# yang-0201/MAF-YOLO

Measured on AMD Instinct MI355X. Metric: images/sec MAF-YOLO-n 640x640 bs=32 infer (Model.forward + non_max_suppression), higher is better.
Workload: dtype f16

## Files before the change

### maf-yolo_amd/csrc/bottleneck.hip

```cpp
#include "maf_common.h"
#include "lds_pipe.h"

namespace {

struct BnArgs {
    const half_t* x; half_t* out;
    const unsigned char* par;
    const float* b2;
    int B, H, W, Cin, Cout, nMB, x_stride, x_coff, out_stride, out_coff;
    int tilesX, tilesY, nwg;
    int ko;
    const half_t* xs[3];
    int xs_stride[3], xs_coff[3];
    const unsigned char* w3;
    int C3, nx;
    unsigned* ctr;
    int ntiles;
    unsigned long long* prof;
};

#ifdef MAF_BN_PROFILE
#define BN_KO(bit) ((a.ko >> (bit)) & 1)
#else
#define BN_KO(bit) 0
#endif
#ifdef MAF_BN_STAMPS
#define BN_STAMP(i) do { uint64_t now_; asm volatile("s_memtime %0\n\ts_waitcnt lgkmcnt(0)" : "=s"(now_) :: "memory"); prof_acc[i] += (uint32_t)(now_ - prof_t); prof_t = now_; } while (0)
#else
#define BN_STAMP(i) do { } while (0)
#endif

typedef half_t half4v_t __attribute__((ext_vector_type(4)));


__device__ __forceinline__ float bn_silu2(float v) { return v * __builtin_amdgcn_rcpf(1.f + __builtin_amdgcn_exp2f(-v)); }
__device__ __forceinline__ void bn_silu2_pk4(float v0, float v1, float v2, float v3, half2_t& o01, half2_t& o23) {
    const half2_t xa = {(half_t)v0, (half_t)v1}, xb = {(half_t)v2, (half_t)v3};
    const uint32_t ua = __builtin_bit_cast(uint32_t, xa), ub = __builtin_bit_cast(uint32_t, xb);
    uint32_t ea, eb, ra, rb;
    asm("v_exp_f16_sdwa %0, -%1 dst_sel:WORD_0 dst_unused:UNUSED_PAD src0_sel:WORD_0" : "=v"(ea) : "v"(ua));
    asm("v_exp_f16_sdwa %0, -%1 dst_sel:WORD_0 dst_unused:UNUSED_PAD src0_sel:WORD_0" : "=v"(eb) : "v"(ub));
    asm("v_exp_f16_sdwa %0, -%1 dst_sel:WORD_1 dst_unused:UNUSED_PRESERVE src0_sel:WORD_1" : "+v"(ea) : "v"(ua));
    asm("v_exp_f16_sdwa %0, -%1 dst_sel:WORD_1 dst_unused:UNUSED_PRESERVE src0_sel:WORD_1" : "+v"(eb) : "v"(ub));
    const half2_t one = {(half_t)1.f, (half_t)1.f};
    const uint32_t da = __builtin_bit_cast(uint32_t, __builtin_bit_cast(half2_t, ea) + one), db = __builtin_bit_cast(uint32_t, __builtin_bit_cast(half2_t, eb) + one);
    asm("v_rcp_f16_sdwa %0, %1 dst_sel:WORD_0 dst_unused:UNUSED_PAD src0_sel:WORD_0" : "=v"(ra) : "v"(da));
    asm("v_rcp_f16_sdwa %0, %1 dst_sel:WORD_0 dst_unused:UNUSED_PAD src0_sel:WORD_0" : "=v"(rb) : "v"(db));
    asm("v_rcp_f16_sdwa %0, %1 dst_sel:WORD_1 dst_unused:UNUSED_PRESERVE src0_sel:WORD_1" : "+v"(ra) : "v"(da));
    asm("v_rcp_f16_sdwa %0, %1 dst_sel:WORD_1 dst_unused:UNUSED_PRESERVE src0_sel:WORD_1" : "+v"(rb) : "v"(db));
    o01 = xa * __builtin_bit_cast(half2_t, ra);
    o23 = xb * __builtin_bit_cast(half2_t, rb);
}
#ifdef MAF_BN_PERSIST
constexpr bool BN_PERSIST = true;
#else
constexpr bool BN_PERSIST = false;
#endif
#ifdef MAF_BN_PKSILU
constexpr bool BN_PK = true;
#else
constexpr bool BN_PK = false;
#endif

template <int K, int S1, int CT2>
struct BnCfg {
    static constexpr int P = K / 2, PARTS = K > 5 ? 2 : 1;
    static constexpr int RH = 16 + K - 1;
    static constexpr int RWC = (16 + K - 1 + 3) & ~3;
    static constexpr int NHP = RH * RWC, NPT = (NHP + 15) / 16;
    static constexpr int MT = (NPT + 3) / 4;
    static constexpr int RWP = 24;
    static constexpr int PSB = ((RH * RWP * 2 - 8 + 255) / 256) * 256 + 8;
    static constexpr int PS = PSB / 2;
    static constexpr int NTOE = 8 * K * PARTS * 16;
    static constexpr int OFF_W1 = 0, OFF_B1 = 2 * S1 * 1024, REC_A = OFF_B1 + 128;
    static constexpr int OFF_TOE = REC_A, OFF_W2 = OFF_TOE + NTOE * 16, OFF_BD = OFF_W2 + CT2 * 1024;
    static constexpr int REC = OFF_BD + 128;
    static constexpr int REC_B = REC - REC_A;
#ifdef MAF_BN_OCC3
    static constexpr bool OCC3 = true;
#else
    static constexpr bool OCC3 = false;
#endif
    static constexpr bool ZT = CT2 == 4 && K <= 5 && !OCC3;
    static constexpr bool DB = !OCC3;
    static constexpr size_t LDS = (size_t)32 * PSB + (size_t)REC + (DB ? (size_t)REC_B : 0) + (ZT ? (size_t)NTOE * 16 : 0);
    static constexpr int ZOFF = REC + (DB ? REC_B : 0);
};

template <int K, int S1, int CT2, int C3T = 0, int NX = 0>
__global__ __launch_bounds__(256, ((CT2 == 2 && K <= 5) || (BnCfg<K, S1, CT2>::OCC3 && K <= 5)) ? 3 : 2) void bottleneck_kernel(const BnArgs a) {
    typedef BnCfg<K, S1, CT2> Cf;
    constexpr int P = Cf::P, PARTS = Cf::PARTS, RWC = Cf::RWC, NHP = Cf::NHP, NPT = Cf::NPT, MT = Cf::MT, RWP = Cf::RWP, PS = Cf::PS;
    extern __shared__ __attribute__((aligned(16))) unsigned char smem_raw[];
    half_t* T1 = reinterpret_cast<half_t*>(smem_raw);
    unsigned char* rec = smem_raw + 32 * Cf::PSB;

    const int tid = threadIdx.x, wave = tid >> 6, lane = tid & 63, g = lane >> 4, p = lane & 15;
    int lid;
    __shared__ int s_next;
    const int my_xcd = blockIdx.x & 7;
    const int seg_q = a.ntiles >> 3, seg_r = a.ntiles & 7;
    auto seg_start = [&](int x) { return x < seg_r ? x * (seg_q + 1) : seg_r * (seg_q + 1) + (x - seg_r) * seg_q; };
    auto seg_stat = [&](int x) { return ((int)gridDim.x >> 3) + (x < ((int)gridDim.x & 7) ? 1 : 0); };
    auto fetch_tile = [&]() -> int {
        const int j = seg_stat(my_xcd) + (int)atomicAdd(a.ctr + my_xcd, 1u);
        return j < seg_q + (my_xcd < seg_r ? 1 : 0) ? seg_start(my_xcd) + j : -1;
    };
    {
        const int bid = blockIdx.x, xcd = bid & 7, j = bid >> 3;
        const int q = a.ntiles >> 3, r = a.ntiles & 7;
        lid = (xcd < r ? xcd * (q + 1) : r * (q + 1) + (xcd - r) * q) + j;
    }
    bool first_tile = true;
    for (;;) {
    int tid_l = threadIdx.x;
    if constexpr (BN_PERSIST) asm volatile("" : "+v"(tid_l));
    const int tid = tid_l, wave = tid >> 6, lane = tid & 63, g = lane >> 4, p = lane & 15;
    int next_tile = -1;
    if (BN_PERSIST && tid == 0) next_tile = fetch_tile();
    const int tx = lid % a.tilesX;
    const int tt = lid / a.tilesX;
    const int ty = tt % a.tilesY;
    const int b = tt / a.tilesY;
    const int y0 = ty * 16, x0 = tx * 16;
    const half_t* xin = a.x + (size_t)b * a.H * a.W * a.x_stride + a.x_coff;

    const int cg0 = g * 8 < a.Cin ? g * 8 : 0;
    const int cg1 = 32 + g * 8 < a.Cin ? 32 + g * 8 : 0;
    uint32_t xoff[MT];
#pragma unroll
    for (int i = 0; i < MT; ++i) {
        const int m = (wave + 4 * i) * 16 + p;
        const int hr = m / RWC, hc = m - hr * RWC;
        const int iy = min(max(y0 - P + hr, 0), a.H - 1), ix = min(max(x0 - P + hc, 0), a.W - 1);
        xoff[i] = (uint32_t)(iy * a.W + ix) * a.x_stride;
    }
    int ko_block = 0;
#ifndef MAF_BN_XD
#define MAF_BN_XD 3
#endif
    constexpr int XD = Cf::OCC3 ? 1 : (MAF_BN_XD < MT ? MAF_BN_XD : MT - 1);
    half8_t af[XD + 1][S1];
    auto load_x = [&](auto idx) {
        constexpr int i = decltype(idx)::value;
        if constexpr (i < MT) {
            if (BN_KO(0) && ko_block > 0) return;
            af[i % (XD + 1)][0] = *reinterpret_cast<const half8_t*>(xin + xoff[i] + cg0);
            if constexpr (S1 > 1) af[i % (XD + 1)][1] = *reinterpret_cast<const half8_t*>(xin + xoff[i] + cg1);
        }
    };
    auto load_x_head = [&]() {
        maf_static_for<XD>([&](auto idx) { load_x(idx); });
    };
    const bool interior = y0 - P >= 0 && x0 - P >= 0 && y0 - P + Cf::RH <= a.H && x0 - P + RWC <= a.W;
    constexpr int MTH = Cf::OCC3 ? 1 : MT;
    uint32_t tmlo[MTH], tmhi[MTH];
    int tdst[MTH];
#pragma unroll
    for (int i = 0; i < (Cf::OCC3 ? 0 : MT); ++i) {
        const int m0 = (wave + 4 * i) * 16 + g * 4;
        const int hr = m0 / RWC, hc0 = m0 - hr * RWC;
        tmlo[i] = tmhi[i] = 0xffffffffu;
        if (!interior) {
            const int iy = y0 - P + hr, ixb = x0 - P + hc0;
            const bool rowok = (unsigned)iy < (unsigned)a.H;
            const uint32_t k0 = (rowok && (unsigned)(ixb + 0) < (unsigned)a.W) ? 0x0000ffffu : 0u, k1 = (rowok && (unsigned)(ixb + 1) < (unsigned)a.W) ? 0xffff0000u : 0u;
            const uint32_t k2 = (rowok && (unsigned)(ixb + 2) < (unsigned)a.W) ? 0x0000ffffu : 0u, k3 = (rowok && (unsigned)(ixb + 3) < (unsigned)a.W) ? 0xffff0000u : 0u;
            tmlo[i] = k0 | k1; tmhi[i] = k2 | k3;
        }
        tdst[i] = m0 < NHP ? p * PS + hr * RWP + hc0 : -1;
    }
    auto dma_part = [&](int mb, int off, int bytes, int dst) {
        const unsigned char* src = a.par + (size_t)mb * Cf::REC + off;
        const int nvec = bytes >> 4;
        for (int v0 = wave * 64; v0 < nvec; v0 += 256) {
            if (v0 + lane < nvec)
                __builtin_amdgcn_global_load_lds((const void __attribute__((address_space(1)))*)(src + (size_t)(v0 + lane) * 16),
                                                 (void __attribute__((address_space(3)))*)(rec + dst + v0 * 16), 16, 0, 0);
        }
    };

    f32x4_t acc2[4][CT2];
#pragma unroll
    for (int i = 0; i < 4; ++i)
#pragma unroll
        for (int ct = 0; ct < CT2; ++ct) acc2[i][ct] = (f32x4_t)0.f;

    const uint32_t toe_mask = (p >> 2) == g ? 0xffffffffu : 0u;
    const int q4 = wave * 4;
    int hi_off = 4;
    asm volatile("" : "+v"(hi_off));

#ifdef MAF_BN_STAMPS
    uint32_t prof_acc[8] = {0, 0, 0, 0, 0, 0, 0, 0};
    uint64_t prof_t;
    asm volatile("s_memtime %0\n\ts_waitcnt lgkmcnt(0)" : "=s"(prof_t) :: "memory");
#endif
    dma_part(0, 0, Cf::REC, 0);
    load_x_head();
    if constexpr (Cf::ZT) {
        if (first_tile) {
            u32x4_t* z = reinterpret_cast<u32x4_t*>(rec + Cf::ZOFF);
            for (int i = tid; i < Cf::NTOE; i += 256) z[i] = (u32x4_t){0u, 0u, 0u, 0u};
        }
    }
    __syncthreads();
    BN_STAMP(0);

    for (int mb = 0; mb < a.nMB; ++mb) {
        ko_block = mb;
        if (!Cf::DB && mb > 0) dma_part(mb, Cf::REC_A, Cf::REC_B, Cf::REC_A);
        const unsigned char* recB = rec + (Cf::DB ? (mb & 1) * Cf::REC_B : 0);
        if (!BN_KO(8)) {
            half8_t w1f[2][S1];
#pragma unroll
            for (int ct = 0; ct < 2; ++ct)
#pragma unroll
                for (int ks = 0; ks < S1; ++ks) w1f[ct][ks] = reinterpret_cast<const half8_t*>(rec + Cf::OFF_W1)[(ct * S1 + ks) * 64 + lane];
            const float b1v0 = reinterpret_cast<const float*>(rec + Cf::OFF_B1)[p], b1v1 = reinterpret_cast<const float*>(rec + Cf::OFF_B1)[16 + p];
            f32x4_t accn[2];
            auto mma_tile = [&](auto idx) {
                constexpr int i = decltype(idx)::value;
                if constexpr (i < MT) {
                    accn[0] = (f32x4_t)b1v0; accn[1] = (f32x4_t)b1v1;
#pragma unroll
                    for (int ks = 0; ks < S1; ++ks)
#pragma unroll
                        for (int ct = 0; ct < 2; ++ct) {
                            const half8_t wv = Cf::OCC3 ? reinterpret_cast<const half8_t*>(rec + Cf::OFF_W1)[(ct * S1 + ks) * 64 + lane] : w1f[ct][ks];
                            accn[ct] = __builtin_amdgcn_mfma_f32_16x16x32_f16(af[i % (XD + 1)][ks], wv, accn[ct], 0, 0, 0);
                        }
                }
            };
            if constexpr (!Cf::OCC3) mma_tile(std::integral_constant<int, 0>{});
            maf_static_for<MT>([&](auto idx) {
                constexpr int i = decltype(idx)::value;
                const int t = wave + 4 * i;
                load_x(std::integral_constant<int, i + XD>{});
                if constexpr (Cf::OCC3) mma_tile(idx);
                f32x4_t acc1[2] = {accn[0], accn[1]};
                if constexpr (!Cf::OCC3) mma_tile(std::integral_constant<int, i + 1>{});
                __builtin_amdgcn_sched_barrier(0);
                uint32_t mlo, mhi;
                int doff;
                if constexpr (!Cf::OCC3) {
                    mlo = tmlo[i]; mhi = tmhi[i]; doff = tdst[i];
                } else {
                    const int m0 = t * 16 + g * 4;
                    const int hr = m0 / RWC, hc0 = m0 - hr * RWC;
                    mlo = mhi = 0xffffffffu;
                    if (!interior) {
                        const int iy = y0 - P + hr, ixb = x0 - P + hc0;
                        const bool rowok = (unsigned)iy < (unsigned)a.H;
                        mlo = ((rowok && (unsigned)(ixb + 0) < (unsigned)a.W) ? 0x0000ffffu : 0u) | ((rowok && (unsigned)(ixb + 1) < (unsigned)a.W) ? 0xffff0000u : 0u);
                        mhi = ((rowok && (unsigned)(ixb + 2) < (unsigned)a.W) ? 0x0000ffffu : 0u) | ((rowok && (unsigned)(ixb + 3) < (unsigned)a.W) ? 0xffff0000u : 0u);
                    }
                    doff = m0 < NHP ? p * PS + hr * RWP + hc0 : -1;
                }
                half_t* dst = T1 + doff;
#pragma unroll
                for (int ct = 0; ct < 2; ++ct) {
                    half2_t h01, h23;
                    if (BN_KO(1)) {
                        h01 = half2_t{(half_t)acc1[ct][0], (half_t)acc1[ct][1]}; h23 = half2_t{(half_t)acc1[ct][2], (half_t)acc1[ct][3]};
                    } else if constexpr (BN_PK) {
                        bn_silu2_pk4(acc1[ct][0], acc1[ct][1], acc1[ct][2], acc1[ct][3], h01, h23);
                    } else {
                        h01 = half2_t{(half_t)bn_silu2(acc1[ct][0]), (half_t)bn_silu2(acc1[ct][1])};
                        h23 = half2_t{(half_t)bn_silu2(acc1[ct][2]), (half_t)bn_silu2(acc1[ct][3])};
                    }
                    const u32x2_t w = {__builtin_bit_cast(uint32_t, h01) & mlo, __builtin_bit_cast(uint32_t, h23) & mhi};
                    if (doff >= 0 && !BN_KO(4)) *reinterpret_cast<u32x2_t*>(dst + (size_t)(16 * ct) * PS) = w;
                }
            });
        }
        BN_STAMP(1);
        if (!BN_KO(7)) __syncthreads();
        BN_STAMP(2);
        if (mb + 1 < a.nMB) {
            if (!BN_KO(5)) {
            dma_part(mb + 1, 0, Cf::REC_A, 0);
            if (Cf::DB) dma_part(mb + 1, Cf::REC_A, Cf::REC_B, Cf::REC_A + ((mb + 1) & 1) * Cf::REC_B);
            }
            load_x_head();
        }

        f32x4_t dacc[8];
        {
            const f32x4_t bd0 = reinterpret_cast<const f32x4_t*>(recB + Cf::OFF_BD)[g * 2], bd1 = reinterpret_cast<const f32x4_t*>(recB + Cf::OFF_BD)[g * 2 + 1];
#pragma unroll
            for (int s = 0; s < 4; ++s) { dacc[s] = (f32x4_t)bd0[s]; dacc[4 + s] = (f32x4_t)bd1[s]; }
        }
        const half8_t* toe = reinterpret_cast<const half8_t*>(recB + Cf::OFF_TOE) + p;
        const half_t* t1l = T1 + (size_t)g * PS + p * RWP + q4;
        const half_t* t1h = t1l + hi_off;
#ifdef MAF_BN_B128
        constexpr bool B128 = true;
#else
        constexpr bool B128 = false;
#endif
        constexpr int NSTEP = K * PARTS * 8, BD = (CT2 == 2 || Cf::OCC3) ? 2 : 3;
        u32x4_t avr[BD + 1];
        u32x4_t bwin[BD + 1];
        u32x2_t blo[BD + 1], bhi[BD + 1];
        const half8_t* toe_src = toe;
        if constexpr (Cf::ZT) { if (!toe_mask) toe_src = reinterpret_cast<const half8_t*>(rec + Cf::ZOFF) + p; }
        const uint32_t a_toe = (uint32_t)(uintptr_t)(const __attribute__((address_space(3))) void*)toe_src;
        const uint32_t a_t1l = (uint32_t)(uintptr_t)(const __attribute__((address_space(3))) void*)t1l;
        const uint32_t a_t1h = (uint32_t)(uintptr_t)(const __attribute__((address_space(3))) void*)t1h;
        auto ld_step = [&](auto idx) {
            constexpr int t = decltype(idx)::value;
            if constexpr (t < NSTEP) {
                constexpr int s = t % 8, part = (t / 8) % PARTS, ky = t / (8 * PARTS);
                constexpr int ot = ((s * K + ky) * PARTS + part) * 256, o = (s * 4 * PS + ky * RWP + part * 4) * 2;
                static_assert(ot < 65536 && o < 65536, "ds offset field");
                lp_ds_read_b128<ot>(avr[t % (BD + 1)], a_toe);
                if constexpr (B128) {
                    lp_ds_read_b128<o>(bwin[t % (BD + 1)], a_t1l);
                } else {
                    lp_ds_read_b64<o>(blo[t % (BD + 1)], a_t1l);
                    lp_ds_read_b64<o>(bhi[t % (BD + 1)], a_t1h);
                }
            }
        };
        lp_wait_lgkm<0>();
        if (!BN_KO(2)) {
        maf_static_for<BD>([&](auto idx) { ld_step(idx); });
        maf_static_for<NSTEP>([&](auto idx) {
            constexpr int t = decltype(idx)::value, s = t % 8, sl = t % (BD + 1);
            ld_step(std::integral_constant<int, t + BD>{});
            constexpr int ahead = (NSTEP - 1 - t) < BD ? (NSTEP - 1 - t) : BD;
            u32x4_t bw;
            if constexpr (B128) {
                lp_wait_lgkm<2 * ahead>(avr[sl], bwin[sl]);
                bw = bwin[sl];
            } else {
                lp_wait_lgkm<3 * ahead>(avr[sl], blo[sl], bhi[sl]);
                bw = (u32x4_t){blo[sl][0], blo[sl][1], bhi[sl][0], bhi[sl][1]};
            }
            const u32x4_t am = Cf::ZT ? avr[sl] : (avr[sl] & toe_mask);
            dacc[s] = __builtin_amdgcn_mfma_f32_16x16x32_f16(__builtin_bit_cast(half8_t, am), __builtin_bit_cast(half8_t, bw), dacc[s], 0, 0, 0);
            __builtin_amdgcn_sched_barrier(0);
        });
        }
        BN_STAMP(3);
        {
            half8_t w2f[CT2];
#pragma unroll
            for (int ct = 0; ct < CT2; ++ct) w2f[ct] = reinterpret_cast<const half8_t*>(recB + Cf::OFF_W2)[ct * 64 + lane];
#pragma unroll
            for (int r = 0; r < 4; ++r) {
                half8_t t2;
#pragma unroll
                for (int s = 0; s < 8; ++s) t2[s] = (half_t)dacc[s][r];
                if (!BN_KO(3)) {
                    if constexpr (BN_PK) {
#pragma unroll
                        for (int s = 0; s < 8; s += 4) {
                            half2_t ha, hb;
                            bn_silu2_pk4(dacc[s][r], dacc[s + 1][r], dacc[s + 2][r], dacc[s + 3][r], ha, hb);
                            t2[s] = ha[0]; t2[s + 1] = ha[1]; t2[s + 2] = hb[0]; t2[s + 3] = hb[1];
                        }
                    } else {
#pragma unroll
                        for (int s = 0; s < 8; ++s) t2[s] = (half_t)bn_silu2(dacc[s][r]);
                    }
                }
#pragma unroll
                for (int ct = 0; ct < CT2; ++ct) if (!BN_KO(9)) {
                    if constexpr (C3T > 0) acc2[r][ct] = __builtin_amdgcn_mfma_f32_16x16x32_f16(w2f[ct], t2, acc2[r][ct], 0, 0, 0);
                    else acc2[r][ct] = __builtin_amdgcn_mfma_f32_16x16x32_f16(t2, w2f[ct], acc2[r][ct], 0, 0, 0);
                }
            }
        }
        BN_STAMP(4);
        if (mb + 1 < a.nMB && !BN_KO(7)) {
            __syncthreads();
        }
        BN_STAMP(5);
    }

    if constexpr (C3T > 0) {
    constexpr int YS = CT2 / 2, NV = 4 * C3T, PSZ = (NV % 8 == 0) ? 8 : 4, NPC = NV / PSZ, NXS = NX * S1, NFR = (NXS + YS) * C3T;
    static_assert(NFR * 1024 + 64 * C3T <= (int)Cf::LDS, "the tail's record fits the LDS of the block loop");
    static_assert((NFR - 1) * 1024 < 65536, "ds offset field");
    __syncthreads();
    {
        constexpr int nvec = (NFR * 1024 + 64 * C3T) >> 4;
        for (int v0 = wave * 64; v0 < nvec; v0 += 256)
            if (v0 + lane < nvec)
                __builtin_amdgcn_global_load_lds((const void __attribute__((address_space(1)))*)(a.w3 + (size_t)(v0 + lane) * 16),
                                                 (void __attribute__((address_space(3)))*)(smem_raw + v0 * 16), 16, 0, 0);
    }
    const int oy = y0 + p, oyc = min(oy, a.H - 1);
    const size_t rowpix = ((size_t)b * a.H + oyc) * a.W;
    int cgk[S1];
#pragma unroll
    for (int ks = 0; ks < S1; ++ks) cgk[ks] = 32 * ks + 8 * g < a.Cin ? 32 * ks + 8 * g : 0;
    half8_t xf[2][2][S1];
    auto load_item = [&](auto idx) {
        constexpr int i = decltype(idx)::value;
        if constexpr (i < 2 * NX) {
            constexpr int h = i / NX, sx = i % NX;
#pragma unroll
            for (int rl = 0; rl < 2; ++rl) {
                const int oxc = min(x0 + q4 + 2 * h + rl, a.W - 1);
                const half_t* px = a.xs[sx] + (rowpix + oxc) * a.xs_stride[sx] + a.xs_coff[sx];
#pragma unroll
                for (int ks = 0; ks < S1; ++ks) xf[i & 1][rl][ks] = *reinterpret_cast<const half8_t*>(px + cgk[ks]);
            }
        }
    };
    load_item(std::integral_constant<int, 0>{});
    half8_t yf[4][YS];
    {
        float b2v[4 * CT2];
#pragma unroll
        for (int i = 0; i < 4 * CT2; ++i) b2v[i] = a.b2[g * 4 * CT2 + i];
#pragma unroll
        for (int r = 0; r < 4; ++r)
#pragma unroll
            for (int j = 0; j < YS; ++j)
#pragma unroll
                for (int q = 0; q < 8; ++q) {
                    const int idx = 8 * j + q, rr = idx / CT2, ct = idx % CT2;
                    yf[r][j][q] = (half_t)maf_act<MAF_ACT_SILU>(acc2[r][ct][rr] + b2v[idx]);
                }
    }
    lp_wait_vm<0>();
    __syncthreads();
    const uint32_t a_w3 = (uint32_t)(uintptr_t)(const __attribute__((address_space(3))) void*)(smem_raw + lane * 16);
    const f32x4_t* b3l = reinterpret_cast<const f32x4_t*>(smem_raw + NFR * 1024) + g * C3T;
    half_t* obase = a.out + a.out_coff + g * PSZ;
    maf_static_for<2>([&](auto hidx) {
        constexpr int h = decltype(hidx)::value;
        f32x4_t acc3[2][C3T];
#pragma unroll
        for (int t3 = 0; t3 < C3T; ++t3) { acc3[0][t3] = b3l[t3]; acc3[1][t3] = acc3[0][t3]; }
        auto group = [&](auto base_c, auto nks_c, auto&& getB) {
            constexpr int FB = decltype(base_c)::value, NKS = decltype(nks_c)::value, NST = NKS * C3T, RD = NST > 4 ? 4 : NST - 1;
            u32x4_t wr[RD + 1];
            auto ld = [&](auto idx) {
                constexpr int t = decltype(idx)::value;
                if constexpr (t < NST) lp_ds_read_b128<(FB + t) * 1024>(wr[t % (RD + 1)], a_w3);
            };
            lp_wait_lgkm<0>();
            maf_static_for<RD>([&](auto idx) { ld(idx); });
            maf_static_for<NST>([&](auto idx) {
                constexpr int t = decltype(idx)::value, ks = t / C3T, t3 = t % C3T, sl = t % (RD + 1);
                ld(std::integral_constant<int, t + RD>{});
                constexpr int ahead = (NST - 1 - t) < RD ? (NST - 1 - t) : RD;
                lp_wait_lgkm<ahead>(wr[sl]);
                const half8_t wv = __builtin_bit_cast(half8_t, wr[sl]);
                acc3[0][t3] = __builtin_amdgcn_mfma_f32_16x16x32_f16(wv, getB(0, ks), acc3[0][t3], 0, 0, 0);
                acc3[1][t3] = __builtin_amdgcn_mfma_f32_16x16x32_f16(wv, getB(1, ks), acc3[1][t3], 0, 0, 0);
                __builtin_amdgcn_sched_barrier(0);
            });
        };
        maf_static_for<NX>([&](auto sidx) {
            constexpr int sx = decltype(sidx)::value, i = h * NX + sx;
            load_item(std::integral_constant<int, i + 1>{});
            group(std::integral_constant<int, sx * S1 * C3T>{}, std::integral_constant<int, S1>{}, [&](int rl, int ks) { return xf[i & 1][rl][ks]; });
        });
        group(std::integral_constant<int, NXS * C3T>{}, std::integral_constant<int, YS>{}, [&](int rl, int j) { return yf[2 * h + rl][j]; });
        if (!BN_KO(6)) {
#pragma unroll
        for (int rl = 0; rl < 2; ++rl) {
            const int ox = x0 + q4 + 2 * h + rl;
            if (oy < a.H && ox < a.W) {
                half_t* op = obase + (((size_t)b * a.H + oy) * a.W + ox) * a.out_stride;
#pragma unroll
                for (int pc = 0; pc < NPC; ++pc) {
                    uint32_t w[PSZ / 2];
#pragma unroll
                    for (int e = 0; e < PSZ / 2; ++e) {
                        const int v0 = pc * PSZ + 2 * e, v1 = v0 + 1;
                        const half2_t hv = {(half_t)maf_act<MAF_ACT_SILU>(acc3[rl][v0 % C3T][v0 / C3T]), (half_t)maf_act<MAF_ACT_SILU>(acc3[rl][v1 % C3T][v1 / C3T])};
                        w[e] = __builtin_bit_cast(uint32_t, hv);
                    }
                    if constexpr (PSZ == 8) *reinterpret_cast<u32x4_t*>(op + pc * 32) = (u32x4_t){w[0], w[1], w[2 % (PSZ / 2)], w[3 % (PSZ / 2)]};
                    else *reinterpret_cast<u32x2_t*>(op + pc * 16) = (u32x2_t){w[0], w[1]};
                }
            }
        }
        }
    });
    } else {
    float bias2[CT2];
#pragma unroll
    for (int ct = 0; ct < CT2; ++ct) bias2[ct] = a.b2[p * CT2 + ct];
    constexpr int CO = 16 * CT2;
    static_assert(4 * 64 * CO * 2 <= 32 * Cf::PSB, "epilogue staging fits the T1 area");
    __syncthreads();
    half_t* stg = T1 + wave * (64 * CO);
#pragma unroll
    for (int r = 0; r < 4; ++r) {
#pragma unroll
        for (int rr = 0; rr < 4; ++rr) {
            uint32_t w[CT2 / 2];
#pragma unroll
            for (int c2 = 0; c2 < CT2 / 2; ++c2) {
                const half2_t h = {(half_t)maf_act<MAF_ACT_SILU>(acc2[r][2 * c2][rr] + bias2[2 * c2]),
                                   (half_t)maf_act<MAF_ACT_SILU>(acc2[r][2 * c2 + 1][rr] + bias2[2 * c2 + 1])};
                w[c2] = __builtin_bit_cast(uint32_t, h);
            }
            half_t* sp = stg + ((g * 4 + rr) * 4 + r) * CO + p * CT2;
            if (CT2 == 4) *reinterpret_cast<u32x2_t*>(sp) = (u32x2_t){w[0], w[1 % (CT2 / 2)]};
            else *reinterpret_cast<uint32_t*>(sp) = w[0];
        }
    }
    const int cpp = a.Cout >> 3;
    half_t* obase = a.out + (size_t)b * a.H * a.W * a.out_stride + a.out_coff;
    if (!BN_KO(6)) {
    for (int q = lane; q < 64 * cpp; q += 64) {
        const int px = q / cpp, part = q - px * cpp;
        const int oy = y0 + (px >> 2), ox = x0 + q4 + (px & 3);
        if (oy < a.H && ox < a.W)
            *reinterpret_cast<u32x4_t*>(obase + ((size_t)oy * a.W + ox) * a.out_stride + 8 * part) = *reinterpret_cast<const u32x4_t*>(stg + px * CO + 8 * part);
    }
    }
    }
    if constexpr (!BN_PERSIST) break;
    __syncthreads();
    if (tid == 0) s_next = next_tile;
    __syncthreads();
    lid = s_next;
    first_tile = false;
    if (lid < 0) break;
    }
    if (BN_PERSIST && tid == 0) {
        __threadfence();
        if (atomicAdd(a.ctr + 8, 1u) == gridDim.x - 1) {
            for (int i = 0; i < 9; ++i) atomicExch(a.ctr + i, 0u);
        }
    }
#ifdef MAF_BN_STAMPS
    BN_STAMP(6);
    if (a.prof && lane == 0)
        for (int i = 0; i < 7; ++i) atomicAdd(a.prof + i, (unsigned long long)prof_acc[i]);
#endif
}

template <int K, int S1, int CT2, int C3T = 0, int NX = 0>
int launch_one(const BnArgs& a, hipStream_t s) {
    constexpr size_t lds = BnCfg<K, S1, CT2>::LDS;
    static_assert(lds <= 160 * 1024, "bottleneck: LDS budget");
    static bool attr = false;
    if (!attr && lds > 64 * 1024) {
        int rc = maf_check_hip(hipFuncSetAttribute(reinterpret_cast<const void*>(&bottleneck_kernel<K, S1, CT2, C3T, NX>),
                                                   hipFuncAttributeMaxDynamicSharedMemorySize, (int)lds), "hipFuncSetAttribute(bottleneck)");
        if (rc) return rc;
        attr = true;
    }
    int grid = a.nwg;
    BnArgs b = a;
    if (BN_PERSIST) {
        static int per_cu = 0;
        static unsigned* ctrs = nullptr;
        static unsigned seq = 0;
        if (!per_cu) {
            int n = 0;
            if (maf_check_hip(hipOccupancyMaxActiveBlocksPerMultiprocessor(&n, reinterpret_cast<const void*>(&bottleneck_kernel<K, S1, CT2, C3T, NX>), 256, lds), "occupancy(bottleneck)")) return MAF_E_HIP;
            if (maf_check_hip(hipMalloc(reinterpret_cast<void**>(&ctrs), 64 * 16 * sizeof(unsigned)), "hipMalloc(bottleneck counters)")) return MAF_E_HIP;
            if (maf_check_hip(hipMemset(ctrs, 0, 64 * 16 * sizeof(unsigned)), "hipMemset(bottleneck counters)")) return MAF_E_HIP;
            per_cu = n > 0 ? n : 1;
        }
        const int slots = per_cu * 256;
        if (grid > slots) grid = slots;
        b.ctr = ctrs + (seq++ & 63) * 16;
    }
    hipLaunchKernelGGL((bottleneck_kernel<K, S1, CT2, C3T, NX>), dim3(grid), dim3(256), lds, s, b);
    return maf_check_hip(hipGetLastError(), "bottleneck launch");
}

template <int K>
int launch_k(const BnArgs& a, hipStream_t s) {
    const int s1 = (a.Cin + 31) / 32, ct2 = a.Cout <= 32 ? 2 : 4;
    if (a.w3) {
        const int c3t = a.C3 / 16;
#define BN_TAIL(KK, SS, CC, TT, NN) if constexpr (K == KK) { if (s1 == SS && ct2 == CC && c3t == TT && a.nx == NN) return launch_one<KK, SS, CC, TT, NN>(a, s); }
        BN_TAIL(3, 1, 2, 3, 2) BN_TAIL(5, 2, 4, 6, 2) BN_TAIL(5, 2, 4, 8, 2)
        BN_TAIL(3, 1, 2, 4, 3) BN_TAIL(5, 2, 4, 8, 3) BN_TAIL(3, 2, 4, 6, 3)
#undef BN_TAIL
        maf_set_error("bottleneck: no instantiation with the fused closing conv for this (k, c, C3, sources)");
        return MAF_E_UNSUPPORTED;
    }
    if (s1 == 1 && ct2 == 2) return launch_one<K, 1, 2>(a, s);
    if (s1 == 2 && ct2 == 4) return launch_one<K, 2, 4>(a, s);
    maf_set_error("bottleneck: unsupported channel count");
    return MAF_E_UNSUPPORTED;
}

}

extern "C" int64_t maf_bottleneck_tail_record_bytes(int32_t c, int32_t nsrc, int32_t c3) {
    const int s1 = (c + 31) / 32, ys = c <= 32 ? 1 : 2, c3t = c3 / 16;
    if (c3 % 16 || nsrc < 2 || nsrc > 3) return 0;
    return (int64_t)(nsrc * s1 + ys) * c3t * 1024 + 64 * c3t;
}

extern "C" int maf_bottleneck_tail_supported(int32_t k, int32_t c, int32_t nsrc, int32_t c3) {
    const int s1 = (c + 31) / 32, ct2 = c <= 32 ? 2 : 4, t = c3 / 16;
    if (c3 % 16 || c % 8 || c > 64) return 0;
    return (k == 3 && s1 == 1 && ct2 == 2 && t == 3 && nsrc == 2) || (k == 5 && s1 == 2 && ct2 == 4 && (t == 6 || t == 8) && nsrc == 2)
        || (k == 3 && s1 == 1 && ct2 == 2 && t == 4 && nsrc == 3) || (k == 5 && s1 == 2 && ct2 == 4 && t == 8 && nsrc == 3) || (k == 3 && s1 == 2 && ct2 == 4 && t == 6 && nsrc == 3);
}

extern "C" int64_t maf_bottleneck_record_bytes(int32_t k, int32_t cin, int32_t cout) {
    const int parts = k > 5 ? 2 : 1, s1 = (cin + 31) / 32, ct2 = cout <= 32 ? 2 : 4;
    return (int64_t)8 * k * parts * 16 * 16 + (int64_t)2 * s1 * 1024 + (int64_t)ct2 * 1024 + 256;
}

int maf_launch_bottleneck(const maf_op_t* op, hipStream_t s) {
    MAF_REQUIRE(op->dtype == MAF_F16, "bottleneck: fp16 only (the fp32 parity mode runs the three kernels separately)");
    const maf_src_t& sr = op->src[0];
    const bool tail = op->nc > 0;
    MAF_REQUIRE((tail ? (op->nsrc == 2 || op->nsrc == 3) : op->nsrc == 1) && sr.mode == MAF_SRC_DIRECT && sr.ptr && op->out, "bottleneck: one direct source (nc > 0: + the other 1 or 2 concat sources of the closing conv)");
    MAF_REQUIRE(op->Cin % 8 == 0 && op->Cin <= 64 && op->Cout % 8 == 0 && op->Cout <= 64, "bottleneck: c <= 64 channels in and out, multiples of 8");
    MAF_REQUIRE(sr.stride % 8 == 0 && sr.coff % 8 == 0 && op->out_stride % 8 == 0 && op->out_coff % 8 == 0, "bottleneck: stride/offset alignment (16-byte pieces)");
    MAF_REQUIRE(op->act == MAF_ACT_SILU, "bottleneck: DepthBottleneckUni applies SiLU after every stage (common.py:918-927)");
    MAF_REQUIRE(op->tile_k > 0 && op->w && op->bias, "bottleneck: null weights (w = block records, bias = b2), tile_k = 32-channel mid blocks");
    BnArgs a;
    a.x = static_cast<const half_t*>(sr.ptr); a.out = static_cast<half_t*>(op->out);
    a.par = static_cast<const unsigned char*>(op->w); a.b2 = op->bias;
    a.B = op->B; a.H = op->H; a.W = op->W; a.Cin = op->Cin; a.Cout = op->Cout; a.nMB = op->tile_k;
    a.x_stride = sr.stride; a.x_coff = sr.coff; a.out_stride = op->out_stride; a.out_coff = op->out_coff;
    a.tilesX = maf_cdiv(a.W, 16); a.tilesY = maf_cdiv(a.H, 16);
    a.nwg = a.B * a.tilesX * a.tilesY;
    a.ntiles = a.nwg; a.ctr = nullptr;
    a.prof = nullptr; a.ko = 0;
    a.w3 = nullptr; a.C3 = 0; a.nx = 0;
    for (int i = 0; i < 3; ++i) { a.xs[i] = nullptr; a.xs_stride[i] = a.xs_coff[i] = 0; }
    if (tail) {
        MAF_REQUIRE(op->aux[0] && op->nc % 16 == 0, "bottleneck: nc > 0 needs aux[0] = the closing conv's record and nc a multiple of 16");
        a.nx = op->nsrc; a.C3 = op->nc; a.w3 = static_cast<const unsigned char*>(op->aux[0]);
        for (int i = 0; i < op->nsrc; ++i) {
            const maf_src_t& q = op->src[i == op->nsrc - 1 ? 0 : i + 1];
            MAF_REQUIRE(q.ptr && q.mode == MAF_SRC_DIRECT && q.C == op->Cin && q.stride % 8 == 0 && q.coff % 8 == 0, "bottleneck: concat sources of the closing conv are direct, Cin channels each, 16-byte aligned");
            a.xs[i] = static_cast<const half_t*>(q.ptr); a.xs_stride[i] = q.stride; a.xs_coff[i] = q.coff;
        }
    }
#ifdef MAF_BN_PROFILE
    a.prof = const_cast<unsigned long long*>(static_cast<const unsigned long long*>(op->aux[3]));
    a.ko = (int)(intptr_t)op->aux[2];
#endif
    switch (op->ksize) {
        case 3: return launch_k<3>(a, s);
        case 5: return launch_k<5>(a, s);
        case 7: return launch_k<7>(a, s);
        case 9: return launch_k<9>(a, s);
        default: maf_set_error("bottleneck: k must be 3, 5, 7 or 9"); return MAF_E_UNSUPPORTED;
    }
}
```

### maf-yolo_amd/csrc/lds_pipe.h

```cpp
#pragma once
#include "maf_common.h"

template <int OFF> __device__ __forceinline__ void lp_ds_read_b128(u32x4_t& d, uint32_t addr) { asm volatile("ds_read_b128 %0, %1 offset:%2" : "=v"(d) : "v"(addr), "n"(OFF)); }
template <int OFF> __device__ __forceinline__ void lp_ds_read_b64(u32x2_t& d, uint32_t addr) { asm volatile("ds_read_b64 %0, %1 offset:%2" : "=v"(d) : "v"(addr), "n"(OFF)); }

template <int N, typename A> __device__ __forceinline__ void lp_wait_lgkm(A& a) { asm volatile("s_waitcnt lgkmcnt(%1)" : "+v"(a) : "n"(N)); }
template <int N, typename A, typename B> __device__ __forceinline__ void lp_wait_lgkm(A& a, B& b) { asm volatile("s_waitcnt lgkmcnt(%2)" : "+v"(a), "+v"(b) : "n"(N)); }
template <int N, typename A, typename B, typename C> __device__ __forceinline__ void lp_wait_lgkm(A& a, B& b, C& c) { asm volatile("s_waitcnt lgkmcnt(%3)" : "+v"(a), "+v"(b), "+v"(c) : "n"(N)); }
template <int N> __device__ __forceinline__ void lp_wait_lgkm() { asm volatile("s_waitcnt lgkmcnt(%0)" ::"n"(N) : "memory"); }
template <int N> __device__ __forceinline__ void lp_wait_vm() { asm volatile("s_waitcnt vmcnt(%0)" ::"n"(N) : "memory"); }

__device__ __forceinline__ uint32_t lp_lds_addr(const void* p) { return (uint32_t)(uintptr_t)(const __attribute__((address_space(3))) void*)p; }
```

Baseline: 17210.

## Keep all input tiles resident, mask toeplitz LDS reads, optionally prefetch tail weights

The bottleneck kernel can now load every input x fragment for a tile up front into registers (RESX) instead of software-pipelining them with a lookahead depth. It also adds a DIAG mode that reads the depthwise toeplitz weights with an exec-masked ds_read so that only the diagonal lanes load data, replacing the AND mask and the extra zeroed LDS copy. An optional EARLY3 path, off by default, prefetches part of the tail 1x1 weights into the spare double-buffer slot. The aim is less load latency and less LDS traffic and footprint, at the cost of more VGPRs, which may lower occupancy.

```diff
diff --git a/maf-yolo_amd/csrc/bottleneck.hip b/maf-yolo_amd/csrc/bottleneck.hip
--- a/maf-yolo_amd/csrc/bottleneck.hip
+++ b/maf-yolo_amd/csrc/bottleneck.hip
@@ -61,6 +61,17 @@
 #else
 constexpr bool BN_PK = false;
 #endif
+
+#ifndef MAF_BN_RESX
+#define MAF_BN_RESX 1
+#endif
+#ifndef MAF_BN_DIAG
+#define MAF_BN_DIAG 1
+#endif
+#ifndef MAF_BN_EARLY3
+#define MAF_BN_EARLY3 0
+#endif
+#define MAF_BN_RESX_WHERE (K <= 5 || S1 == 1)
 
 template <int K, int S1, int CT2>
 struct BnCfg {
@@ -82,7 +93,10 @@
 #else
     static constexpr bool OCC3 = false;
 #endif
-    static constexpr bool ZT = CT2 == 4 && K <= 5 && !OCC3;
+    static constexpr bool RESX = !OCC3 && (MAF_BN_RESX == 2 || (MAF_BN_RESX == 1 && MAF_BN_RESX_WHERE));
+    static constexpr bool ZT_FITS = CT2 == 4 && K <= 5 && !OCC3;
+    static constexpr bool DIAG = MAF_BN_DIAG == 2 || (MAF_BN_DIAG == 1 && !ZT_FITS);
+    static constexpr bool ZT = ZT_FITS && !DIAG;
     static constexpr bool DB = !OCC3;
     static constexpr size_t LDS = (size_t)32 * PSB + (size_t)REC + (DB ? (size_t)REC_B : 0) + (ZT ? (size_t)NTOE * 16 : 0);
     static constexpr int ZOFF = REC + (DB ? REC_B : 0);
@@ -95,6 +109,9 @@
     extern __shared__ __attribute__((aligned(16))) unsigned char smem_raw[];
     half_t* T1 = reinterpret_cast<half_t*>(smem_raw);
     unsigned char* rec = smem_raw + 32 * Cf::PSB;
+    constexpr int NFR3 = C3T > 0 ? (NX * S1 + CT2 / 2) * C3T : 0, NE3 = NFR3 < Cf::REC_B / 1024 ? NFR3 : Cf::REC_B / 1024;
+    constexpr bool EARLY3 = MAF_BN_EARLY3 && C3T > 0 && Cf::DB && (NFR3 - NE3) * 1024 + 64 * C3T <= 32 * Cf::PSB + Cf::REC_A;
+    constexpr int NE = EARLY3 ? NE3 : 0;
 
     const int tid = threadIdx.x, wave = tid >> 6, lane = tid & 63, g = lane >> 4, p = lane & 15;
     int lid;
@@ -141,17 +158,19 @@
 #define MAF_BN_XD 3
 #endif
     constexpr int XD = Cf::OCC3 ? 1 : (MAF_BN_XD < MT ? MAF_BN_XD : MT - 1);
-    half8_t af[XD + 1][S1];
+    constexpr bool RESX = Cf::RESX;
+    constexpr int NAF = RESX ? MT : XD + 1;
+    half8_t af[NAF][S1];
     auto load_x = [&](auto idx) {
         constexpr int i = decltype(idx)::value;
         if constexpr (i < MT) {
             if (BN_KO(0) && ko_block > 0) return;
-            af[i % (XD + 1)][0] = *reinterpret_cast<const half8_t*>(xin + xoff[i] + cg0);
-            if constexpr (S1 > 1) af[i % (XD + 1)][1] = *reinterpret_cast<const half8_t*>(xin + xoff[i] + cg1);
+            af[i % NAF][0] = *reinterpret_cast<const half8_t*>(xin + xoff[i] + cg0);
+            if constexpr (S1 > 1) af[i % NAF][1] = *reinterpret_cast<const half8_t*>(xin + xoff[i] + cg1);
         }
     };
     auto load_x_head = [&]() {
-        maf_static_for<XD>([&](auto idx) { load_x(idx); });
+        maf_static_for<RESX ? MT : XD>([&](auto idx) { load_x(idx); });
     };
     const bool interior = y0 - P >= 0 && x0 - P >= 0 && y0 - P + Cf::RH <= a.H && x0 - P + RWC <= a.W;
     constexpr int MTH = Cf::OCC3 ? 1 : MT;
@@ -188,6 +207,13 @@
         for (int ct = 0; ct < CT2; ++ct) acc2[i][ct] = (f32x4_t)0.f;
 
     const uint32_t toe_mask = (p >> 2) == g ? 0xffffffffu : 0u;
+    constexpr uint64_t toe_lanes = (0xFull << 0) | (0xFull << 20) | (0xFull << 40) | (0xFull << 60);
+    constexpr int BD = (CT2 == 2 || Cf::OCC3) ? 2 : 3;
+    u32x4_t avr[BD + 1];
+    if constexpr (Cf::DIAG) {
+#pragma unroll
+        for (int i = 0; i <= BD; ++i) avr[i] = (u32x4_t){0u, 0u, 0u, 0u};
+    }
     const int q4 = wave * 4;
     int hi_off = 4;
     asm volatile("" : "+v"(hi_off));
@@ -229,7 +255,7 @@
 #pragma unroll
                         for (int ct = 0; ct < 2; ++ct) {
                             const half8_t wv = Cf::OCC3 ? reinterpret_cast<const half8_t*>(rec + Cf::OFF_W1)[(ct * S1 + ks) * 64 + lane] : w1f[ct][ks];
-                            accn[ct] = __builtin_amdgcn_mfma_f32_16x16x32_f16(af[i % (XD + 1)][ks], wv, accn[ct], 0, 0, 0);
+                            accn[ct] = __builtin_amdgcn_mfma_f32_16x16x32_f16(af[i % NAF][ks], wv, accn[ct], 0, 0, 0);
                         }
                 }
             };
@@ -237,7 +263,7 @@
             maf_static_for<MT>([&](auto idx) {
                 constexpr int i = decltype(idx)::value;
                 const int t = wave + 4 * i;
-                load_x(std::integral_constant<int, i + XD>{});
+                if constexpr (!RESX) load_x(std::integral_constant<int, i + XD>{});
                 if constexpr (Cf::OCC3) mma_tile(idx);
                 f32x4_t acc1[2] = {accn[0], accn[1]};
                 if constexpr (!Cf::OCC3) mma_tile(std::integral_constant<int, i + 1>{});
@@ -283,7 +309,12 @@
             dma_part(mb + 1, 0, Cf::REC_A, 0);
             if (Cf::DB) dma_part(mb + 1, Cf::REC_A, Cf::REC_B, Cf::REC_A + ((mb + 1) & 1) * Cf::REC_B);
             }
-            load_x_head();
+            if constexpr (!RESX) load_x_head();
+        } else if constexpr (NE > 0) {
+            unsigned char* e3 = rec + Cf::REC_A + (a.nMB & 1) * Cf::REC_B;
+            for (int v0 = wave * 64; v0 < NE * 64; v0 += 256)
+                __builtin_amdgcn_global_load_lds((const void __attribute__((address_space(1)))*)(a.w3 + (size_t)(v0 + lane) * 16),
+                                                 (void __attribute__((address_space(3)))*)(e3 + v0 * 16), 16, 0, 0);
         }
 
         f32x4_t dacc[8];
@@ -300,8 +331,7 @@
 #else
         constexpr bool B128 = false;
 #endif
-        constexpr int NSTEP = K * PARTS * 8, BD = (CT2 == 2 || Cf::OCC3) ? 2 : 3;
-        u32x4_t avr[BD + 1];
+        constexpr int NSTEP = K * PARTS * 8;
         u32x4_t bwin[BD + 1];
         u32x2_t blo[BD + 1], bhi[BD + 1];
         const half8_t* toe_src = toe;
@@ -315,7 +345,8 @@
                 constexpr int s = t % 8, part = (t / 8) % PARTS, ky = t / (8 * PARTS);
                 constexpr int ot = ((s * K + ky) * PARTS + part) * 256, o = (s * 4 * PS + ky * RWP + part * 4) * 2;
                 static_assert(ot < 65536 && o < 65536, "ds offset field");
-                lp_ds_read_b128<ot>(avr[t % (BD + 1)], a_toe);
+                if constexpr (Cf::DIAG) lp_ds_read_b128_masked<ot>(avr[t % (BD + 1)], a_toe, toe_lanes);
+                else lp_ds_read_b128<ot>(avr[t % (BD + 1)], a_toe);
                 if constexpr (B128) {
                     lp_ds_read_b128<o>(bwin[t % (BD + 1)], a_t1l);
                 } else {
@@ -339,7 +370,7 @@
                 lp_wait_lgkm<3 * ahead>(avr[sl], blo[sl], bhi[sl]);
                 bw = (u32x4_t){blo[sl][0], blo[sl][1], bhi[sl][0], bhi[sl][1]};
             }
-            const u32x4_t am = Cf::ZT ? avr[sl] : (avr[sl] & toe_mask);
+            const u32x4_t am = (Cf::ZT || Cf::DIAG) ? avr[sl] : (avr[sl] & toe_mask);
             dacc[s] = __builtin_amdgcn_mfma_f32_16x16x32_f16(__builtin_bit_cast(half8_t, am), __builtin_bit_cast(half8_t, bw), dacc[s], 0, 0, 0);
             __builtin_amdgcn_sched_barrier(0);
         });
@@ -385,12 +416,14 @@
     constexpr int YS = CT2 / 2, NV = 4 * C3T, PSZ = (NV % 8 == 0) ? 8 : 4, NPC = NV / PSZ, NXS = NX * S1, NFR = (NXS + YS) * C3T;
     static_assert(NFR * 1024 + 64 * C3T <= (int)Cf::LDS, "the tail's record fits the LDS of the block loop");
     static_assert((NFR - 1) * 1024 < 65536, "ds offset field");
+    static_assert(NFR == NFR3 && NE <= NFR, "fragment count of the record");
     __syncthreads();
     {
-        constexpr int nvec = (NFR * 1024 + 64 * C3T) >> 4;
+        constexpr int nvec = ((NFR - NE) * 1024 + 64 * C3T) >> 4;
+        const unsigned char* src = a.w3 + NE * 1024;
         for (int v0 = wave * 64; v0 < nvec; v0 += 256)
             if (v0 + lane < nvec)
-                __builtin_amdgcn_global_load_lds((const void __attribute__((address_space(1)))*)(a.w3 + (size_t)(v0 + lane) * 16),
+                __builtin_amdgcn_global_load_lds((const void __attribute__((address_space(1)))*)(src + (size_t)(v0 + lane) * 16),
                                                  (void __attribute__((address_space(3)))*)(smem_raw + v0 * 16), 16, 0, 0);
     }
     const int oy = y0 + p, oyc = min(oy, a.H - 1);
@@ -431,7 +464,8 @@
     lp_wait_vm<0>();
     __syncthreads();
     const uint32_t a_w3 = (uint32_t)(uintptr_t)(const __attribute__((address_space(3))) void*)(smem_raw + lane * 16);
-    const f32x4_t* b3l = reinterpret_cast<const f32x4_t*>(smem_raw + NFR * 1024) + g * C3T;
+    const uint32_t a_w3e = lp_lds_addr(rec + Cf::REC_A + (a.nMB & 1) * Cf::REC_B + lane * 16);
+    const f32x4_t* b3l = reinterpret_cast<const f32x4_t*>(smem_raw + (NFR - NE) * 1024) + g * C3T;
     half_t* obase = a.out + a.out_coff + g * PSZ;
     maf_static_for<2>([&](auto hidx) {
         constexpr int h = decltype(hidx)::value;
@@ -443,7 +477,10 @@
             u32x4_t wr[RD + 1];
             auto ld = [&](auto idx) {
                 constexpr int t = decltype(idx)::value;
-                if constexpr (t < NST) lp_ds_read_b128<(FB + t) * 1024>(wr[t % (RD + 1)], a_w3);
+                if constexpr (t < NST) {
+                    if constexpr (FB + t < NE) lp_ds_read_b128<(FB + t) * 1024>(wr[t % (RD + 1)], a_w3e);
+                    else lp_ds_read_b128<(FB + t - NE) * 1024>(wr[t % (RD + 1)], a_w3);
+                }
             };
             lp_wait_lgkm<0>();
             maf_static_for<RD>([&](auto idx) { ld(idx); });
diff --git a/maf-yolo_amd/csrc/lds_pipe.h b/maf-yolo_amd/csrc/lds_pipe.h
--- a/maf-yolo_amd/csrc/lds_pipe.h
+++ b/maf-yolo_amd/csrc/lds_pipe.h
@@ -3,6 +3,9 @@
 
 template <int OFF> __device__ __forceinline__ void lp_ds_read_b128(u32x4_t& d, uint32_t addr) { asm volatile("ds_read_b128 %0, %1 offset:%2" : "=v"(d) : "v"(addr), "n"(OFF)); }
 template <int OFF> __device__ __forceinline__ void lp_ds_read_b64(u32x2_t& d, uint32_t addr) { asm volatile("ds_read_b64 %0, %1 offset:%2" : "=v"(d) : "v"(addr), "n"(OFF)); }
+template <int OFF> __device__ __forceinline__ void lp_ds_read_b128_masked(u32x4_t& d, uint32_t addr, uint64_t mask) {
+    asm volatile("s_mov_b64 exec, %2\n\tds_read_b128 %0, %1 offset:%3\n\ts_mov_b64 exec, -1" : "+v"(d) : "v"(addr), "s"(mask), "n"(OFF));
+}
 
 template <int N, typename A> __device__ __forceinline__ void lp_wait_lgkm(A& a) { asm volatile("s_waitcnt lgkmcnt(%1)" : "+v"(a) : "n"(N)); }
 template <int N, typename A, typename B> __device__ __forceinline__ void lp_wait_lgkm(A& a, B& b) { asm volatile("s_waitcnt lgkmcnt(%2)" : "+v"(a), "+v"(b) : "n"(N)); }
```

Measured after the change: 17250, median of 2. Within noise of the previous version (+0.2%).
